# GrumpyZhou/patch2pix

Hardware: AMD Instinct MI355X
Metric: image-pairs/sec (480x640, ptmax=400), matching hot path, feature pyramids resident in HBM (higher is better)
Workload: dtype f32-equivalent: fp16x2 (every f32 operand, scaled by an exact power of two, = sum of 2 fp16 planes to within 2^-24 of its magnitude; 3 fp16 MFMA products per f32 product, f32 accumulate); second convolution as Winograd F(2x2,3x3) (transforms in f32, filters transformed in f64)

## Files before the change

### patch2pix_amd/csrc/regress_common.h

```cpp
#pragma once
#include "p2p_common.h"
#include <algorithm>
#include <cmath>
#include <cstring>
#include <vector>

namespace p2p {

constexpr int NT = 512;
constexpr int MAXB = 16;

struct RegDev {
    const float *wp1, *wp2;
    const float *wh1, *wh2;
    const float *bn1s, *bn1b, *bn2s, *bn2b;
    const float *bn1s_h, *bn2s_h;
    const float *fc1t, *fc1b, *bnf1s, *bnf1b, *fc2t, *fc2b, *bnf2s, *bnf2b, *fc3, *fc3b;
    const float *fc1p, *fc2p;
    const float *ww2, *bn2s_w;
};

struct ItemDev {
    const float *pyr[2][4];
    int H[2], W[2];
};

struct RegressArgs {
    ItemDev item[MAXB];
    int start[MAXB + 1];
    const int *dev_counts;
    int nitems;
    const void *proposals;
    int is_float, n, nlevels;
    RegDev reg[2];
    float *matches[2], *probs[2], *raw[2];
    float *ws;
    unsigned char *wU;
    float *hinv;
    int lvl0, p0, p1, mblocks;
};
static_assert(sizeof(RegDev) == 24 * sizeof(void *) && sizeof(RegressArgs) == 1864, "kernel-argument layout of the fine stage");

constexpr int FC_ROWS = 16;
constexpr int WINO_BLK = 16384;
#ifndef P2P_WINO_CHUNK
#define P2P_WINO_CHUNK 3328
#endif
constexpr int WINO_CHUNK = P2P_WINO_CHUNK;
static_assert(WINO_CHUNK % 256 == 0 && WINO_CHUNK >= 256, "chunks are whole units of 256 proposals");
static inline int wino_nchunks(size_t n) {
    const size_t units = (n + 255) / 256, per = WINO_CHUNK / 256;
    return (int)std::max<size_t>(1, (units + per - 1) / per);
}
static inline void wino_chunk_range(size_t n, int c, int *p0, int *p1) {
    const size_t units = (n + 255) / 256, nch = (size_t)wino_nchunks(n), base = units / nch, rem = units % nch;
    const size_t u0 = (size_t)c * base + std::min<size_t>((size_t)c, rem), u1 = u0 + base + ((size_t)c < rem ? 1 : 0);
    *p0 = (int)std::min(n, u0 * 256);
    *p1 = (int)std::min(n, u1 * 256);
}
static inline size_t regress_ws_base_floats(size_t n) { return ((2 * n * 512 + 31) & ~size_t(31)) + 4 * n + 32; }
static inline size_t wino_hinv_offset_floats(size_t n) { return (regress_ws_base_floats(n) + 63) & ~size_t(63); }
static inline size_t wino_chunk_rows(size_t n) {
    return (std::min(n, (size_t)WINO_CHUNK) + 7) & ~size_t(7);
}
static inline size_t wino_u_offset_floats(size_t n) { return (wino_hinv_offset_floats(n) + wino_chunk_rows(n) + 63) & ~size_t(63); }
static inline size_t regress_ws_floats(size_t n) {
    return wino_u_offset_floats(n) + (size_t)16 * (wino_chunk_rows(n) / 8) * 16 * (WINO_BLK / 4);
}

__device__ __forceinline__ int clampi(int v, int lo, int hi) { return v < lo ? lo : (v > hi ? hi : v); }

__device__ __forceinline__ int level_dim(int dim, int j) { return (dim + (1 << j) - 1) >> j; }

__device__ __forceinline__ int patch_cell(int origin, int p, int j, int dim) {
    const int d = dim >> j;
    return clampi((origin + p) >> j, 0, d - 1) - clampi(origin >> j, 0, d - 1);
}

template <class A>
__device__ __forceinline__ int wino_slot(const A &a, int c) {
    if (!a.dev_counts) return c < a.n ? c : -1;
    int cum = 0;
    for (int it = 0; it < a.nitems; ++it) {
        const int cnt = max(0, min(a.dev_counts[it], a.start[it + 1] - a.start[it]));
        if (c < cum + cnt) return a.start[it] + (c - cum);
        cum += cnt;
    }
    return -1;
}

__device__ __forceinline__ void fc_tail_parse(const RegDev &R, const ItemDev &I, const RegressArgs &args, int lvl, int prop,
                                              int tid, const float *V, float *F1, float *F2, float *misc) {
    P2P_OPAQUE(tid);
    {
        const f32x4 *w = (const f32x4 *)R.fc1t + tid;
        float s = 0.f;
#pragma unroll 1
        for (int k0 = 0; k0 < 128; k0 += 32) {
            f32x4 wv[32];
#pragma unroll
            for (int i = 0; i < 32; ++i) wv[i] = w[(k0 + i) * 512];
#pragma unroll
            for (int i = 0; i < 32; ++i) {
                const f32x4 x = *(const f32x4 *)(V + 4 * (k0 + i));
                s = fmaf(wv[i][0], x[0], s);
                s = fmaf(wv[i][1], x[1], s);
                s = fmaf(wv[i][2], x[2], s);
                s = fmaf(wv[i][3], x[3], s);
            }
        }
        s += R.fc1b[tid];
        F1[tid] = fmaxf(fmaf(s, R.bnf1s[tid], R.bnf1b[tid]), 0.f);
    }
    __syncthreads();
    if (tid < 256) {
        const f32x4 *w = (const f32x4 *)R.fc2t + tid;
        float s = 0.f;
#pragma unroll 1
        for (int k0 = 0; k0 < 128; k0 += 32) {
            f32x4 wv[32];
#pragma unroll
            for (int i = 0; i < 32; ++i) wv[i] = w[(k0 + i) * 256];
#pragma unroll
            for (int i = 0; i < 32; ++i) {
                const f32x4 x = *(const f32x4 *)(F1 + 4 * (k0 + i));
                s = fmaf(wv[i][0], x[0], s);
                s = fmaf(wv[i][1], x[1], s);
                s = fmaf(wv[i][2], x[2], s);
                s = fmaf(wv[i][3], x[3], s);
            }
        }
        s += R.fc2b[tid];
        F2[tid] = fmaxf(fmaf(s, R.bnf2s[tid], R.bnf2b[tid]), 0.f);
    }
    __syncthreads();
    if (tid < 5) {
        const f32x4 *w = (const f32x4 *)(R.fc3 + tid * 256);
        float s = 0.f;
#pragma unroll 1
        for (int k0 = 0; k0 < 64; k0 += 16) {
            f32x4 wv[16];
#pragma unroll
            for (int i = 0; i < 16; ++i) wv[i] = w[k0 + i];
#pragma unroll
            for (int i = 0; i < 16; ++i) {
                const f32x4 x = *(const f32x4 *)(F2 + 4 * (k0 + i));
                s = fmaf(wv[i][0], x[0], s);
                s = fmaf(wv[i][1], x[1], s);
                s = fmaf(wv[i][2], x[2], s);
                s = fmaf(wv[i][3], x[3], s);
            }
        }
        s += R.fc3b[tid];
        misc[tid] = s;
        if (args.raw[lvl]) args.raw[lvl][(size_t)prop * 5 + tid] = s;
        if (tid < 4) {
            const float off = 16.0f * tanhf(fmaxf(s, 0.f)) - 8.0f;
            float fm = misc[8 + tid] + off;
            const float hi = (float)((tid == 0) ? I.W[0] : (tid == 1) ? I.H[0] : (tid == 2) ? I.W[1] : I.H[1]);
            fm = fminf(fmaxf(fm, 0.f), hi);
            if (args.matches[lvl]) args.matches[lvl][(size_t)prop * 4 + tid] = fm;
            misc[8 + tid] = fm;
        } else {
            if (args.probs[lvl]) args.probs[lvl][prop] = 1.0f / (1.0f + expf(-s));
        }
    }
    __syncthreads();
}

__device__ __forceinline__ float load_coherent(const float *p) {
    return __int_as_float(__atomic_load_n((const int *)p, __ATOMIC_RELAXED));
}
#define P2P_MFMA_F32_16(a, b, c) __builtin_amdgcn_mfma_f32_16x16x4f32((a), (b), (c), 0, 0, 0)

constexpr int FCST1 = 512 + 4, FCST2 = 256 + 4;
constexpr int FC_LDS_BYTES = FC_ROWS * (2 * FCST1 + FCST2) * 4;

__device__ __forceinline__ void fc_batch_parse(const RegDev &R, const RegressArgs &args, int lvl, const float *wsV,
                                               float *nextp, unsigned char *smb, int tid) {
    P2P_OPAQUE(tid);
    const int nwg = gridDim.x, first = blockIdx.x;
    const int cnt = (args.n - first + nwg - 1) / nwg;
    const int lane = tid & 63, wave = __builtin_amdgcn_readfirstlane(tid >> 6), l15 = lane & 15, kb = lane >> 4;
    float *Vs = (float *)smb, *F1s = Vs + FC_ROWS * FCST1, *F2s = F1s + FC_ROWS * FCST1;
#pragma unroll 1
    for (int r0 = 0; r0 < cnt; r0 += FC_ROWS) {
        {
            const int row = tid >> 5, c4 = tid & 31;
            const bool ok = r0 + row < cnt;
            const float *src = wsV + (size_t)(first + (r0 + row) * nwg) * 512;
#pragma unroll
            for (int q = 0; q < 4; ++q) {
                const int col = 4 * (c4 + 32 * q);
                f32x4 v = {0.f, 0.f, 0.f, 0.f};
                if (ok) v = (f32x4){load_coherent(src + col), load_coherent(src + col + 1), load_coherent(src + col + 2), load_coherent(src + col + 3)};
                *(f32x4 *)(Vs + row * FCST1 + col) = v;
            }
        }
        __syncthreads();
        {
            f32x4 acc[4];
#pragma unroll
            for (int t = 0; t < 4; ++t) acc[t] = (f32x4){0.f, 0.f, 0.f, 0.f};
            const float *w = R.fc1p + ((size_t)(wave * 4) * 64 + lane) * 4;
            const float *a = Vs + l15 * FCST1 + 4 * kb;
#pragma unroll 2
            for (int S = 0; S < 32; ++S) {
                const f32x4 av = *(const f32x4 *)(a + 16 * S);
                f32x4 bv[4];
#pragma unroll
                for (int t = 0; t < 4; ++t) bv[t] = *(const f32x4 *)(w + ((size_t)S * 32 + t) * 256);
#pragma unroll
                for (int j = 0; j < 4; ++j)
#pragma unroll
                    for (int t = 0; t < 4; ++t) acc[t] = P2P_MFMA_F32_16(av[j], bv[t][j], acc[t]);
            }
#pragma unroll
            for (int t = 0; t < 4; ++t) {
                const int n = 16 * (4 * wave + t) + l15;
                const float b = R.fc1b[n], s = R.bnf1s[n], sh = R.bnf1b[n];
#pragma unroll
                for (int r = 0; r < 4; ++r) F1s[(4 * kb + r) * FCST1 + n] = fmaxf(fmaf(acc[t][r] + b, s, sh), 0.f);
            }
        }
        __syncthreads();
        {
            f32x4 acc[2];
#pragma unroll
            for (int t = 0; t < 2; ++t) acc[t] = (f32x4){0.f, 0.f, 0.f, 0.f};
// ... 184 lines not shown
```

### patch2pix_amd/csrc/regress_h2.hip

```cpp
#define XNPL 2
#include "regress_common.h"

#include <algorithm>
#include <cmath>
#include <vector>

namespace p2p {

typedef _Float16 xe8 __attribute__((ext_vector_type(8)));
typedef _Float16 xe2 __attribute__((ext_vector_type(2)));
typedef float f32x2 __attribute__((ext_vector_type(2)));
constexpr int XUB = XNPL * 1024;

constexpr int XST1 = 64 * 2 + 16;
constexpr int XRP1 = 9 * XST1 + 112;
constexpr int XPL1 = 9 * XRP1;
constexpr int YST2 = 64 * 2 + 16, YNC2 = 25, YPL2 = (YNC2 + 3) * YST2;
constexpr int YST3 = 128 * 2 + 32, YNC3 = 9, YPL3 = (YNC3 + 2) * YST3;
constexpr int XOFF1 = 0;
constexpr int YOFF2 = XOFF1 + XNPL * XPL1;
constexpr int YOFF3 = YOFF2 + XNPL * YPL2;
constexpr int XIMG = YOFF3 + XNPL * YPL3;
constexpr int XRAW0 = 2 * XIMG;
constexpr int XSHARED = XRAW0 + 2 * 3 * 256 * 4;
// ... 16 lines not shown
#ifdef P2P_X3_TIMING
constexpr int XSM_BYTES = XSM_MISC + 16 * 4 + 8 * 16 * 4;
#else
constexpr int XSM_BYTES = XSM_MISC + 16 * 4;
#endif
static_assert(FC_LDS_BYTES <= XSM_MISC, "the FC batch stages its rows over the convolution buffers");
static_assert(XTMP1 + 2 * XTMP1IMG <= XSHR && 64 * XA0ST <= XSHR, "the shared region is sized by the fold buffers");
static_assert(XPL1 % 16 == 0 && XTMP1 % 16 == 0 && XIMG % 16 == 0 && YOFF2 % 16 == 0 && YOFF3 % 16 == 0 && YPL2 % 16 == 0 && YPL3 % 16 == 0 && XSHARED % 16 == 0 &&
              XTAB % 16 == 0 && XSM_SCALE % 16 == 0 && HPL % 16 == 0 && HCHUNK % 16 == 0 && XCONV2B % 16 == 0,
              "16-byte alignment of ds_read_b128");
static_assert(XSM_BYTES <= 160 * 1024, "LDS budget");

__device__ __forceinline__ unsigned pk_e(float a, float b) {
    const f32x2 v = {a, b};
    return __builtin_bit_cast(unsigned, __builtin_convertvector(v, xe2));
}
__device__ __forceinline__ unsigned short f2e(float f) { return __builtin_bit_cast(unsigned short, (_Float16)f); }
__device__ __forceinline__ float e2f(unsigned short b) { return (float)__builtin_bit_cast(_Float16, b); }
__device__ __forceinline__ float pk_lo(unsigned h) { return (float)__builtin_bit_cast(xe2, h)[0]; }
__device__ __forceinline__ float pk_hi(unsigned h) { return (float)__builtin_bit_cast(xe2, h)[1]; }
__device__ __forceinline__ void store_planes(unsigned char *dst, int plane_stride, float v) {
    const unsigned short p0 = f2e(v);
    const float r1 = v - e2f(p0);
    const unsigned short p1 = f2e(r1);
    *(unsigned short *)dst = p0;
    *(unsigned short *)(dst + plane_stride) = p1;
}

__device__ __forceinline__ void splitn(const f32x4 &xa, const f32x4 &xb, float s, f32x4 (&p)[XNPL]) {
    const float x[8] = {xa[0] * s, xa[1] * s, xa[2] * s, xa[3] * s, xb[0] * s, xb[1] * s, xb[2] * s, xb[3] * s};
#pragma unroll
    for (int q = 0; q < 4; ++q) {
        const unsigned h = pk_e(x[2 * q], x[2 * q + 1]);
        const float r0 = x[2 * q] - pk_lo(h);
        const float r1 = x[2 * q + 1] - pk_hi(h);
        const unsigned m = pk_e(r0, r1);
        p[0][q] = __uint_as_float(h);
        p[1][q] = __uint_as_float(m);
    }
}

#ifdef XF_PIN_W
#define XWADV(N)
#else
#define XWADV(N) wb += (N) * XUB;
#endif
#ifdef P2P_X3_TIMING
#define XTL_() ((unsigned *)(smb + XSM_MISC + 64) + wave * 16)
#define XT_START { const unsigned n_ = (unsigned)__builtin_amdgcn_s_memtime(); if (P2P_LANE_ID() < 16) XTL_()[P2P_LANE_ID()] = (P2P_LANE_ID() == 15) ? n_ : 0u; }
#define XT(i) { const unsigned n_ = (unsigned)__builtin_amdgcn_s_memtime(); if (P2P_LANE_ID() == 0) { unsigned *x_ = XTL_(); x_[i] += n_ - x_[15]; x_[15] = n_; } }
#if P2P_X3_TIMING >= 2
#define XTL(i) XT(i)
#else
#define XTL(i)
#endif
#else
#define XT_START
#define XT(i)
#define XTL(i)
#endif
#define XMFMA(a, b, c) __builtin_amdgcn_mfma_f32_32x32x16_f16(__builtin_bit_cast(xe8, (a)), __builtin_bit_cast(xe8, (b)), (c), 0, 0, 0)

#define XLOADR(R, P) R[0] = *(const f32x4 *)(P); R[1] = *(const f32x4 *)((P) + 16);
#define XLOADP(S, P, PL) { _Pragma("unroll") for (int q_ = 0; q_ < XNPL; ++q_) S[q_] = *(const f32x4 *)((P) + q_ * (PL)); }
#define XLOADB(BUF, AHEAD)                                                               \
    { unsigned wo_ = (AHEAD) * XUB; P2P_OPAQUE_S(wo_);          \
      _Pragma("unroll") for (int q_ = 0; q_ < XNPL; ++q_) BUF[q_] = *(const f32x4 *)((wb + wo_) + wlane + q_ * 1024); }
#define XNPROD 3
#define XHALF_(C0IN, C1IN, CU0, CU1, SP, BU0, BU1)                                       \
    CU0 = XMFMA(SP[1], BU0[0], C0IN); CU1 = XMFMA(SP[1], BU1[0], C1IN);                  \
    CU0 = XMFMA(SP[0], BU0[1], CU0); CU1 = XMFMA(SP[0], BU1[1], CU1);                    \
    CU0 = XMFMA(SP[0], BU0[0], CU0); CU1 = XMFMA(SP[0], BU1[0], CU1);
#define XNM (2 * XNPROD)
#define XHALF(CU0, CU1, SP, BU0, BU1) XHALF_(CU0, CU1, CU0, CU1, SP, BU0, BU1)
#define XHALFZ(CU0, CU1, SP, BU0, BU1) XHALF_(zero16, zero16, CU0, CU1, SP, BU0, BU1)

#define XPIPE(NDS)                                                                       \
    __builtin_amdgcn_sched_group_barrier(0x100, NDS, 0); __builtin_amdgcn_sched_group_barrier(0x020, XNPL, 0);        \
    _Pragma("unroll") for (int g_ = 0; g_ < XNM; ++g_) {                                                              \
        __builtin_amdgcn_sched_group_barrier(0x008, 1, 0); __builtin_amdgcn_sched_group_barrier(0x002, 6, 0); }
#define XPIPE0()                                                                         \
    __builtin_amdgcn_sched_group_barrier(0x020, XNPL, 0);                                                             \
    _Pragma("unroll") for (int g_ = 0; g_ < XNM; ++g_) {                                                              \
        __builtin_amdgcn_sched_group_barrier(0x008, 1, 0); __builtin_amdgcn_sched_group_barrier(0x002, 6, 0); }
#define XSLAB(N0, N1, SC0, SC1, BC0, BC1, BN0, BN1, AH)                                   \
    { XLOADR(R0, N0) XLOADB(BN0, AH) splitn(R1[0], R1[1], (SC1), S1);                               \
      XHALF(acc00, acc01, S0, BC0, BC1) XPIPE(2) __builtin_amdgcn_sched_barrier(0);                                   \
      XLOADR(R1, N1) XLOADB(BN1, (AH) + 1) splitn(R0[0], R0[1], (SC0), S0);                          \
      XHALF(acc10, acc11, S1, BC0, BC1) XPIPE(2) __builtin_amdgcn_sched_barrier(0); }
#define XGROUP4(SL0, SL1, SL2, SL3) { SL0 SL1 SL2 SL3 XWADV(8) }
#define XSLABEND(SC1, BC0, BC1, BN0, BN1, AH)                                            \
    { XLOADB(BN0, AH) splitn(R1[0], R1[1], (SC1), S1);                                              \
      XHALF(acc00, acc01, S0, BC0, BC1) XPIPE0() __builtin_amdgcn_sched_barrier(0);                                    \
      XLOADB(BN1, (AH) + 1)                                                                                           \
      XHALF(acc10, acc11, S1, BC0, BC1) XPIPE0() __builtin_amdgcn_sched_barrier(0); }
#define XPRO(P0, P1, SC0) { XLOADR(R0, P0) XLOADR(R1, P1) splitn(R0[0], R0[1], (SC0), S0); }

#define XQHALF_(C0IN, C1IN, CU0, CU1, A0, A1, BU)                                        \
    CU0 = XMFMA(A0[1], BU[0], C0IN); CU1 = XMFMA(A1[1], BU[0], C1IN);                    \
    CU0 = XMFMA(A0[0], BU[1], CU0); CU1 = XMFMA(A1[0], BU[1], CU1);                      \
    CU0 = XMFMA(A0[0], BU[0], CU0); CU1 = XMFMA(A1[0], BU[0], CU1);
#define XQHALF(CU0, CU1, A0, A1, BU) XQHALF_(CU0, CU1, CU0, CU1, A0, A1, BU)
#define XQHALFZ(CU0, CU1, A0, A1, BU) XQHALF_(zero16, zero16, CU0, CU1, A0, A1, BU)
#define XQPIPE()                                                                         \
    _Pragma("unroll") for (int g_ = 0; g_ < 2 * XNPL; ++g_) {                                                        \
        __builtin_amdgcn_sched_group_barrier(0x008, 1, 0); __builtin_amdgcn_sched_group_barrier(0x100, 1, 0); }       \
    __builtin_amdgcn_sched_group_barrier(0x008, 1, 0); __builtin_amdgcn_sched_group_barrier(0x020, XNPL, 0);          \
    __builtin_amdgcn_sched_group_barrier(0x008, 1, 0);
#define XQSTEP(HALF, AC0, AC1, AN0, AN1, NP0, NP1, BC, BN, AH)                            \
    { XLOADP(AN0, NP0, XPL1) XLOADP(AN1, NP1, XPL1) XLOADB(BN, AH)                                                    \
      HALF(tp0, tp1, AC0, AC1, BC) XQPIPE() __builtin_amdgcn_sched_barrier(0); }
#define XPFOLD(ACC0, ACC1)                                                               \
    { _Pragma("unroll") for (int r_ = 0; r_ < 16; ++r_) {                                                             \
          const float e0_ = *(const float *)(tabq + ((2 * (r_ >> 2)) * 17 + 2 * (r_ & 3)) * 8);                       \
          const float e1_ = *(const float *)(tabq + ((8 + 2 * (r_ >> 2)) * 17 + 2 * (r_ & 3)) * 8);                   \
          ACC0[r_] = fmaf(e0_, tp0[r_], ACC0[r_]); ACC1[r_] = fmaf(e1_, tp1[r_], ACC1[r_]); } }

#define XLPIPE(NDS, NMFMA)                                                               \
    __builtin_amdgcn_sched_group_barrier(0x100, NDS, 0); __builtin_amdgcn_sched_group_barrier(0x020, 2 * XNPL, 0);    \
    __builtin_amdgcn_sched_group_barrier(0x008, NMFMA, 0);
#define XCSLAB(HALF, SC, SN, NP, NPL, BC0, BC1, BN0, BN1, AH)                             \
    { XLOADP(SN, NP, NPL) XLOADB(BN0, AH) XLOADB(BN1, (AH) + 1)                                                       \
      HALF(t0, t1, SC, BC0, BC1) XLPIPE(XNPL, XNM) __builtin_amdgcn_sched_barrier(0); }
typedef float f32x4v __attribute__((ext_vector_type(4)));
#define X16MFMA(a, b, c) __builtin_amdgcn_mfma_f32_16x16x32_f16(__builtin_bit_cast(xe8, (a)), __builtin_bit_cast(xe8, (b)), (c), 0, 0, 0)
#define X16HALF_(C0IN, C1IN, CU0, CU1, SP, BU0, BU1)                                     \
    CU0 = X16MFMA(SP[1], BU0[0], C0IN); CU1 = X16MFMA(SP[1], BU1[0], C1IN);              \
    CU0 = X16MFMA(SP[0], BU0[1], CU0); CU1 = X16MFMA(SP[0], BU1[1], CU1);                \
    CU0 = X16MFMA(SP[0], BU0[0], CU0); CU1 = X16MFMA(SP[0], BU1[0], CU1);
#define X16HALF(CU0, CU1, SP, BU0, BU1) X16HALF_(CU0, CU1, CU0, CU1, SP, BU0, BU1)
#define X16HALFZ(CU0, CU1, SP, BU0, BU1) X16HALF_(zero4, zero4, CU0, CU1, SP, BU0, BU1)
#define X16SLAB(HALF, UA, UB, SC, LOADNEXT, BC0, BC1, BN0, BN1, AH)                       \
    { LOADNEXT XLOADB(BN0, AH) XLOADB(BN1, (AH) + 1)                                                                  \
      HALF(UA, UB, SC, BC0, BC1) __builtin_amdgcn_sched_barrier(0); }
#define XPB() { __builtin_amdgcn_sched_barrier(0); __builtin_amdgcn_s_barrier(); __builtin_amdgcn_sched_barrier(0); }
#define XPP() __builtin_amdgcn_sched_barrier(0); __builtin_amdgcn_s_barrier(); __builtin_amdgcn_s_barrier(); __builtin_amdgcn_sched_barrier(0);
#define XHPIPE()                                                                         \
    __builtin_amdgcn_sched_group_barrier(0x008, 2, 0);                                                                \
    _Pragma("unroll") for (int g_ = 0; g_ < 2 * XNPL; ++g_) {                                                        \
        __builtin_amdgcn_sched_group_barrier(0x100, 1, 0); __builtin_amdgcn_sched_group_barrier(0x008, 1, 0); }       \
    _Pragma("unroll") for (int g_ = 0; g_ < 2 * XNPL; ++g_) {                                                        \
        __builtin_amdgcn_sched_group_barrier(0x020, 1, 0); __builtin_amdgcn_sched_group_barrier(0x008, 1, 0); }       \
    __builtin_amdgcn_sched_group_barrier(0x008, 4 * XNPROD - 4 * XNPL - 2, 0);
#define XQUAD(AC0, AC1, BC0, BC1, P, Q)                                                  \
    acc00 = XMFMA(AC0[P], BC0[Q], acc00); acc01 = XMFMA(AC0[P], BC1[Q], acc01);                                       \
    acc11 = XMFMA(AC1[P], BC1[Q], acc11); acc10 = XMFMA(AC1[P], BC0[Q], acc10);
#define XHMFMAS(AC0, AC1, BC0, BC1)                                                      \
    XQUAD(AC0, AC1, BC0, BC1, 1, 0) XQUAD(AC0, AC1, BC0, BC1, 0, 1) XQUAD(AC0, AC1, BC0, BC1, 0, 0)
#define XHSLAB(AC0, AC1, AN0, AN1, NP0, NP1, BC0, BC1, BN0, BN1, AH)                       \
    { XLOADP(AN0, NP0, HPL) XLOADP(AN1, NP1, HPL) XLOADB(BN0, AH) XLOADB(BN1, (AH) + 1)                                \
      XHMFMAS(AC0, AC1, BC0, BC1)                                                                                     \
      XHPIPE() __builtin_amdgcn_sched_barrier(0); }

enum : int {
    MISC_NEXT_PROP = 4,
    MISC_PROP = 8,
    MISC_MIN_SCALE = 12,
    MISC_MAX_H = 14,
};
static_assert(MISC_MAX_H == MISC_MIN_SCALE + 2, "the three reductions are reset by three consecutive threads");

__device__ __forceinline__ int image_exponent(const float *misc, int img) {
    return clampi((((const int *)misc)[MISC_MIN_SCALE + img] >> 23) & 0xff, 13, 240);
}
__device__ __forceinline__ int h_exponent(const float *misc) { return clampi((((const int *)misc)[MISC_MAX_H] >> 23) & 0xff, 20, 250); }
__device__ __forceinline__ float cell_mul(int eb) { return __int_as_float((eb + 12) << 23); }
__device__ __forceinline__ float fold_mul(int eb) { return __int_as_float((254 - eb) << 23); }
__device__ __forceinline__ float h_mul(int eb, int top) { return __int_as_float((254 + top - eb) << 23); }
__device__ __forceinline__ float h_inv(int eb, int top) { return __int_as_float((eb - top) << 23); }

constexpr int level_cells(int j) { return (j == 0) ? 16 : (j == 1) ? 9 : (j == 2) ? 5 : 3; }
constexpr int level_channels(int j) { return (j == 0) ? 3 : (j == 3) ? 128 : 64; }
constexpr int level_loads(int j) { return (level_channels(j) * level_cells(j) * level_cells(j) + NT - 1) / NT; }
__device__ __forceinline__ int tmp_cell(int img, int j, int c) {
    return (j == 1) ? XSHARED + XTMP1 + img * XTMP1IMG + c * XTMP1ST
                    : XSHARED + img * XTMPIMG + ((j == 2) ? c * XTMP2ST : XTMP3 + c * XTMP3ST);
}
__device__ __forceinline__ int opaque_tid(int wave) {
    int t = wave * 64 + P2P_LANE_ID();
    P2P_OPAQUE(t);
    return t;
}
struct GatherRegs { float v[2][4][level_loads(1)]; };
__device__ __forceinline__ void gather_loads(GatherRegs &g, int tv, int xa, int ya, int xb, int yb, const ItemDev &J) {
#pragma unroll
    for (int img = 0; img < 2; ++img) {
        const int Hh = J.H[img], Ww = J.W[img], x0 = img ? xb : xa, y0 = img ? yb : ya;
        {
            const int r0 = clampi(y0, 0, Hh - 1), c0 = clampi(x0, 0, Ww - 1);
            const float *src = J.pyr[img][0];
#pragma unroll
            for (int k = 0; k < level_loads(0); ++k) {
                const int e = tv + k * NT;
                const int c = e >> 8, rem = e & 255, r = rem >> 4, cc = rem & 15;
                g.v[img][0][k] = (e < 768) ? src[((size_t)c * Hh + min(r0 + r, Hh - 1)) * Ww + min(c0 + cc, Ww - 1)] : 0.f;
            }
        }
#pragma unroll
        for (int j = 1; j < 4; ++j) {
            const int Rr = level_cells(j);
            const int Hj = Hh >> j, Wj = Ww >> j;
            const int Ha = level_dim(Hh, j), Wa = level_dim(Ww, j);
            const int r0 = clampi(y0 >> j, 0, Hj - 1);
            const int c0 = clampi(x0 >> j, 0, Wj - 1);
            const float *src = J.pyr[img][j];
#pragma unroll
            for (int k = 0; k < level_loads(j); ++k) {
                const int e = tv + k * NT;
                const int c = e / (Rr * Rr);
                const int rem = e - c * (Rr * Rr);
                const int r = rem / Rr;
                const int cc = rem - r * Rr;
                g.v[img][j][k] = (e < level_channels(j) * Rr * Rr)
                                     ? src[((size_t)c * Ha + min(r0 + r, Hj - 1)) * Wa + min(c0 + cc, Wj - 1)] : 0.f;
            }
        }
    }
}
__device__ __forceinline__ void gather_commit(const GatherRegs &g, int tv, unsigned char *smb) {
#pragma unroll
    for (int img = 0; img < 2; ++img) {
#pragma unroll
        for (int k = 0; k < level_loads(0); ++k) {
            const int e = tv + k * NT;
            if (e < 768) ((float *)(smb + XRAW0))[img * 768 + e] = g.v[img][0][k];
        }
#pragma unroll
        for (int j = 1; j < 4; ++j) {
            const int Rr = level_cells(j);
#pragma unroll
            for (int k = 0; k < level_loads(j); ++k) {
                const int e = tv + k * NT;
                if (e < level_channels(j) * Rr * Rr) {
                    const int c = e / (Rr * Rr);
                    const int rem = e - c * (Rr * Rr);
                    *(float *)(smb + tmp_cell(img, j, rem) + c * 4) = g.v[img][j][k];
                }
            }
        }
    }
}
__device__ __forceinline__ void gather_zero(GatherRegs &g) {
    float zf = 0.f;
    P2P_OPAQUE(zf);
#pragma unroll
    for (int img = 0; img < 2; ++img)
#pragma unroll
        for (int j = 0; j < 4; ++j)
#pragma unroll
            for (int k = 0; k < level_loads(j); ++k) g.v[img][j][k] = zf;
}

#define XWS_V(lvl_) (args.ws + (size_t)(lvl_) * args.n * 512)
#define XWS_NEXTP() (args.ws + ((2 * (size_t)args.n * 512 + 31) & ~(size_t)31))
__device__ __forceinline__ float proposal_coord(const RegressArgs &args, int lvl, int prop, int q) {
    if (lvl > 0) return load_coherent(XWS_NEXTP() + (size_t)prop * 4 + q);
    if (args.is_float) return ((const float *)args.proposals)[(size_t)prop * 4 + q];
    return (float)((const long long *)args.proposals)[(size_t)prop * 4 + q];
}

template <bool WINO>
__global__ __launch_bounds__(NT, 2) void regress_h2_kernel(RegressArgs args) {
    P2P_DYN_SHARED(unsigned char, smb);
    const int tid = threadIdx.x;
    const int wave = __builtin_amdgcn_readfirstlane(tid >> 6);
    const int nwg = gridDim.x;

    float *raw0 = (float *)(smb + XRAW0);
    float *scale = (float *)(smb + XSM_SCALE);
    float *misc = (float *)(smb + XSM_MISC);

#pragma unroll 1
    for (int lvl = WINO ? args.lvl0 : 0; lvl < (WINO ? args.lvl0 + 1 : args.nlevels); ++lvl) {
        const RegDev &R_ = args.reg[lvl];
        GatherRegs gn;
        bool pre = false;
#pragma unroll 1
      for (int cprop = (WINO ? args.p0 : 0) + blockIdx.x; cprop < (WINO ? args.p1 : args.n); cprop += nwg) {
        const int prop = WINO ? wino_slot(args, cprop) : cprop;
        if (WINO && prop < 0) break;
        int it = 0;
        while (it + 1 < args.nitems && prop >= args.start[it + 1]) ++it;
        if (!WINO && args.dev_counts && prop - args.start[it] >= args.dev_counts[it]) continue;
        const ItemDev &I = args.item[it];
        int tq = tid;
        if constexpr (WINO) tq = opaque_tid(wave);
        if (tq < 4) {
            float v = proposal_coord(args, lvl, prop, tq);
#ifdef XF_SAME_PATCH
            v = 100.f + 16.f * tq;
#endif
            misc[MISC_PROP + tq] = v;
        }
        if constexpr (WINO) {
            const int nprop = (cprop + nwg < args.p1) ? wino_slot(args, cprop + nwg) : -1;
            if (nprop >= 0 && tq >= 4 && tq < 8) misc[MISC_NEXT_PROP + tq - 4] = proposal_coord(args, lvl, nprop, tq - 4);
        }
        if (tq >= 64 && tq < 67) ((int *)misc)[MISC_MIN_SCALE + tq - 64] = (tq < 66) ? 0x7f7fffff : 0;
        __syncthreads();
        int moff = MISC_PROP;
        P2P_OPAQUE(moff);
        const int xa = (int)misc[moff + 0] - 8, ya = (int)misc[moff + 1] - 8;
        const int xb = (int)misc[moff + 2] - 8, yb = (int)misc[moff + 3] - 8;
#define XX0(img_) ((img_) ? xb : xa)
#define XY0(img_) ((img_) ? yb : ya)
        const int tidv = opaque_tid(wave);
        const int half = (tidv >> 5) & 1, l31 = tidv & 31;
        XT_START
        if (wave >= 4) __builtin_amdgcn_s_setprio(1);

        if constexpr (WINO) {
            if (!pre) gather_loads(gn, opaque_tid(wave), xa, ya, xb, yb, I);
            gather_commit(gn, opaque_tid(wave), smb);
        } else {
            GatherRegs g;
            gather_loads(g, tidv, xa, ya, xb, yb, I);
            gather_commit(g, tidv, smb);
        }
        if (tidv < 2 * XNPL * (3 * YST2 + 2 * YST3) / 16) {
            const int per = (3 * YST2 + 2 * YST3) / 16;
            const int im = tidv / (XNPL * per), pl = (tidv / per) % XNPL, q = tidv % per;
            float zf = 0.f;
            P2P_OPAQUE(zf);
            unsigned char *z = smb + im * XIMG + ((q < 3 * YST2 / 16) ? YOFF2 + pl * YPL2 + YNC2 * YST2 + q * 16
                                                                      : YOFF3 + pl * YPL3 + YNC3 * YST3 + (q - 3 * YST2 / 16) * 16);
            *(f32x4 *)z = (f32x4){zf, zf, zf, zf};
        }
        __syncthreads();
        XT(0)

        float sc_keep;
        int c23_keep;
        {
            const int img = tidv >> 8, pix = tidv & 255, py = pix >> 4, px = pix & 15;
            float ss = 0.f;
            {
                const float *p = raw0 + img * 768 + patch_cell(XY0(img), py, 0, I.H[img]) * 16 + patch_cell(XX0(img), px, 0, I.W[img]);
#pragma unroll
                for (int c = 0; c < 3; ++c) ss = fmaf(p[c * 256], p[c * 256], ss);
            }
            const int c2 = patch_cell(XY0(img), py, 2, I.H[img]) * 5 + patch_cell(XX0(img), px, 2, I.W[img]);
#pragma unroll
            for (int j = 1; j < 4; ++j) {
                const int cjy = patch_cell(XY0(img), py, j, I.H[img]), cjx = patch_cell(XX0(img), px, j, I.W[img]);
                const unsigned char *p = smb + tmp_cell(img, j, cjy * level_cells(j) + cjx);
                for (int c = 0; c < level_channels(j); c += 4) {
                    const f32x4 v = *(const f32x4 *)(p + c * 4);
                    ss = fmaf(v[0], v[0], ss); ss = fmaf(v[1], v[1], ss); ss = fmaf(v[2], v[2], ss); ss = fmaf(v[3], v[3], ss);
                }
            }
            const float sc = 1.0f / sqrtf(ss + 1e-6f);
            scale[tidv] = sc * 4096.0f;
            atomicMin((int *)misc + MISC_MIN_SCALE + img, __float_as_int(sc));
            sc_keep = sc;
            c23_keep = c2 * XTROW | (patch_cell(XY0(img), py, 3, I.H[img]) * 3 + patch_cell(XX0(img), px, 3, I.W[img])) * XTROW << 16;
            if (tidv < 2 * 33) {
                const int im = tidv / 33, q = tidv - im * 33;
                const int idx = (q < 17) ? q : (q - 16) * 17;
                float zf = 0.f;
                P2P_OPAQUE(zf);
                *(f32x2 *)(smb + XTAB + im * XTABIMG + idx * 8) = (f32x2){zf, zf};
            }
        }
        __syncthreads();
        {
            const int img = tidv >> 8, pix = tidv & 255, py = pix >> 4, px = pix & 15;
            *(f32x2 *)(smb + XTAB + img * XTABIMG + ((py + 1) * 17 + px + 1) * 8) =
                (f32x2){sc_keep * fold_mul(image_exponent(misc, img)), __int_as_float(c23_keep)};
#pragma unroll
            for (int k = 0; k < 11; ++k) {
                const int e = tidv + k * NT;
                if (e < 2 * 2592) {
                    const int im = (e >= 2592), r = e - im * 2592;
                    const float mul = cell_mul(image_exponent(misc, im));
                    const int cell = r >> 5, c2 = (r & 31) * 2, cy = cell / 9, cx = cell - 9 * cy;
                    const f32x2 v = *(const f32x2 *)(smb + tmp_cell(im, 1, cell) + c2 * 4);
                    const unsigned h = pk_e(v[0] * mul, v[1] * mul);
                    unsigned char *d = smb + im * XIMG + XOFF1 + cy * XRP1 + cx * XST1 + c2 * 2;
                    *(unsigned *)d = h;
                    *(unsigned *)(d + XPL1) = pk_e(v[0] * mul - pk_lo(h), v[1] * mul - pk_hi(h));
                }
            }
#pragma unroll
            for (int k = 0; k < 11; ++k) {
                const int e = tidv + k * NT;
                if (e < 2 * 2752) {
                    const int im = (e >= 2752), r = e - im * 2752;
                    const float mul = cell_mul(image_exponent(misc, im));
                    const bool l2 = r < 1600;
                    const int cell = l2 ? r >> 6 : (r - 1600) >> 7, c = l2 ? r & 63 : (r - 1600) & 127;
                    const float v = *(const float *)(smb + tmp_cell(im, l2 ? 2 : 3, cell) + c * 4);
                    store_planes(smb + im * XIMG + (l2 ? YOFF2 + cell * YST2 : YOFF3 + cell * YST3) + c * 2, l2 ? YPL2 : YPL3, v * mul);
                }
            }
        }
        __syncthreads();
        XT(1)

        for (int e = tidv; e < 64 * 64; e += NT) {
            const int m = e >> 6, kk = e & 63, img = kk >> 5, r = kk & 31;
            float v = 0.f;
            if (r < 27) {
                const int tap = r / 3, c = r - tap * 3, ky = tap / 3, kx = tap - ky * 3;
                const int py = 2 * (m >> 3) + ky - 1, px = 2 * (m & 7) + kx - 1;
                if (py >= 0 && px >= 0)
                    v = raw0[img * 768 + c * 256 + patch_cell(XY0(img), py, 0, I.H[img]) * 16 + patch_cell(XX0(img), px, 0, I.W[img])] *
                        scale[img * 256 + py * 16 + px];
            }
            *(float *)(smb + XSHARED + m * XA0ST + kk * 4) = v;
        }
        __syncthreads();
        XT(2)

#define XZERO16(A_) { float z_ = 0.f; P2P_OPAQUE(z_); _Pragma("unroll") for (int i_ = 0; i_ < 16; ++i_) A_[i_] = z_; }
        f32x16 acc00, acc01, acc10, acc11;
        XZERO16(acc00) XZERO16(acc01) XZERO16(acc10) XZERO16(acc11)
        f32x4 B0[XNPL], B1[XNPL], B2[XNPL], B3[XNPL], B4[XNPL], B5[XNPL], B6[XNPL], B7[XNPL], S0[XNPL], S1[XNPL];
        const f32x16 zero16 = {0};
        auto acc_tile = [&](int t, int u) -> const f32x16 & { return (t == 0) ? (u == 0 ? acc00 : acc01) : (u == 0 ? acc10 : acc11); };
        auto bn1_absmax = [&]() {
            float mx = 0.f;
#pragma unroll
            for (int u = 0; u < 2; ++u) {
                const int n = wave * 64 + u * 32 + l31;
                const float s = R_.bn1s_h[n], b = R_.bn1b[n];
#pragma unroll
                for (int t = 0; t < 2; ++t) {
                    const f32x16 &a = acc_tile(t, u);
#pragma unroll
                    for (int r = 0; r < 16; ++r) mx = fmaxf(mx, fabsf(fmaf(a[r], s, b)));
                }
            }
            atomicMax((int *)misc + MISC_MAX_H, __float_as_int(mx));
        };
        {
            f32x4 R0[2], R1[2];
            const unsigned char *wb = (const unsigned char *)R_.wh1 + (size_t)wave * (S1_UNITS + XPF) * XUB;
            const unsigned wlane = (tidv & 63) * 16;
            XLOADB(B0, 0) XLOADB(B1, 1) XLOADB(B2, 2) XLOADB(B3, 3) XLOADB(B4, 4) XLOADB(B5, 5)
            {
                const unsigned char *p0 = smb + XSHARED + l31 * XA0ST + half * 32;
                const unsigned char *p1 = p0 + 32 * XA0ST;
                XPRO(p0, p1, 1.0f)
                XGROUP4(XSLAB(p0 + 64, p1 + 64, 1.0f, 1.0f, B0, B1, B6, B7, 6),
                        XSLAB(p0 + 128, p1 + 128, 1.0f, 1.0f, B2, B3, B0, B1, 8),
                        XSLAB(p0 + 192, p1 + 192, 1.0f, 1.0f, B4, B5, B2, B3, 10),
                        XSLAB(p0, p1, 1.0f, 1.0f, B6, B7, B4, B5, 12))
            }
            __syncthreads();
            XT(3)
            const int c2y = (l31 < 25) ? l31 / 5 : 0, c2x = (l31 < 25) ? l31 - 5 * (l31 / 5) : 0;
            float *Tw = (float *)(smb + XSHARED + (wave & (XT2N - 1)) * XTW) + 2 * l31;
            float *T3w = (float *)(smb + XSHARED + XT2N * XTW + wave * (9 * XTROW));
            const f32x4v zero4 = {0.f, 0.f, 0.f, 0.f};
            const int stagger = wave >> 2;
#pragma unroll 1
            for (int it = 0; it < 18 + stagger; ++it) {
                const int pi = it - stagger;
                if (pi >= 0) {
                    const int tap = pi >> 1, img = pi & 1;
                    const int ky = tap / 3, kx = tap - ky * 3;
                    int ab[2];
#pragma unroll
                    for (int t = 0; t < 2; ++t) {
                        const int p = 32 * t + l31;
                        const int pyc = max(2 * (p >> 3) + ky - 1, 0), pxc = max(2 * (p & 7) + kx - 1, 0);
                        ab[t] = img * XIMG + XOFF1 + patch_cell(XY0(img), pyc, 1, I.H[img]) * XRP1 +
                                patch_cell(XX0(img), pxc, 1, I.W[img]) * XST1 + half * 16;
                    }
                    const unsigned char *a0 = smb + ab[0], *a1 = smb + ab[1];
                    const unsigned char *tabq = smb + XTAB + img * XTABIMG + (ky * 17 + kx + 8 * half) * 8;
#ifdef XF_SKIP_P
                    XWADV(8) (void)a0; (void)a1; (void)tabq;
#else
                    {
                        f32x16 tp0, tp1;
                        XLOADP(S0, a0, XPL1) XLOADP(S1, a1, XPL1)
                        XQSTEP(XQHALFZ, S0, S1, R0, R1, a0 + 32, a1 + 32, B0, B6, 6)
                        XQSTEP(XQHALF, R0, R1, S0, S1, a0 + 64, a1 + 64, B1, B7, 7)
                        XQSTEP(XQHALF, S0, S1, R0, R1, a0 + 96, a1 + 96, B2, B0, 8)
                        XQSTEP(XQHALF, R0, R1, S0, S1, a0, a1, B3, B1, 9)
                        XPFOLD(acc00, acc10)
                        XQSTEP(XQHALFZ, S0, S1, R0, R1, a0 + 32, a1 + 32, B4, B2, 10)
                        XQSTEP(XQHALF, R0, R1, S0, S1, a0 + 64, a1 + 64, B5, B3, 11)
                        XQSTEP(XQHALF, S0, S1, R0, R1, a0 + 96, a1 + 96, B6, B4, 12)
                        XQSTEP(XQHALF, R0, R1, S0, S1, a0 + 96, a1 + 96, B7, B5, 13)
                        XPFOLD(acc01, acc11)
                        XWADV(8)
                    }
#endif
                    XTL(4)
                }
                if (it < 18) {
                    const int tap = it >> 1, img = it & 1;
                    const int ky = tap / 3, kx = tap - ky * 3;
                    int a2, a3;
                    {
                        const int Hh = I.H[img], Ww = I.W[img];
                        const int by2 = clampi(XY0(img) >> 2, 0, (Hh >> 2) - 1), bx2 = clampi(XX0(img) >> 2, 0, (Ww >> 2) - 1);
                        const int by3 = clampi(XY0(img) >> 3, 0, (Hh >> 3) - 1), bx3 = clampi(XX0(img) >> 3, 0, (Ww >> 3) - 1);
                        const int c3y = clampi(min((by2 + c2y) >> 1, (Hh >> 3) - 1) - by3, 0, 2);
                        const int c3x = clampi(min((bx2 + c2x) >> 1, (Ww >> 3) - 1) - bx3, 0, 2);
                        a2 = img * XIMG + YOFF2 + ((l31 < 25) ? (c2y * 5 + c2x) * YST2 + half * 16
                                                              : YNC2 * YST2 + ((((l31 - YNC2) * 9 + half) & 15) << 4));
                        a3 = img * XIMG + YOFF3 + ((l31 < 25) ? c3y * 3 + c3x : YNC3) * YST3 + half * 16;
                    }
                    const unsigned char *q2 = smb + a2, *q3 = smb + a3;
                    f32x16 t0, t1;
#if defined(XF_SKIP_C)
                    t0 = acc00; t1 = acc01; XWADV(24) (void)q2; (void)q3;
#else
                    {
                        (void)q3;
                        const int l16 = (tidv & 15), kb = (tidv >> 4) & 3;
                        const unsigned char *q3r = smb + img * XIMG + YOFF3 + ((l16 < 9) ? l16 * YST3 + kb * 16
                                                                                         : YNC3 * YST3 + (((2 * (l16 - YNC3) + kb) & 15) << 4));
                        f32x4v u0, u1, u2, u3;
                        XLOADP(S0, q3r, YPL3)
                        XGROUP4(X16SLAB(X16HALFZ, u0, u1, S0, XLOADP(S1, q3r + 64, YPL3), B0, B1, B6, B7, 6),
                                X16SLAB(X16HALFZ, u2, u3, S0, , B2, B3, B0, B1, 8),
                                X16SLAB(X16HALF, u0, u1, S1, XLOADP(S0, q3r + 128, YPL3), B4, B5, B2, B3, 10),
                                X16SLAB(X16HALF, u2, u3, S1, , B6, B7, B4, B5, 12))
                        XGROUP4(X16SLAB(X16HALF, u0, u1, S0, XLOADP(S1, q3r + 192, YPL3), B0, B1, B6, B7, 6),
                                X16SLAB(X16HALF, u2, u3, S0, , B2, B3, B0, B1, 8),
                                X16SLAB(X16HALF, u0, u1, S1, XLOADP(S0, q2, YPL2), B4, B5, B2, B3, 10),
                                X16SLAB(X16HALF, u2, u3, S1, , B6, B7, B4, B5, 12))
                        P2P_WAVE_SYNC();
#pragma unroll
                        for (int r = 0; r < 4; ++r)
                            if (4 * kb + r < 9) {
                                f32x2 *d = (f32x2 *)(T3w + (4 * kb + r) * 64) + l16;
                                d[0] = (f32x2){u0[r], u2[r]}; d[16] = (f32x2){u1[r], u3[r]};
                            }
                        XGROUP4(XCSLAB(XHALFZ, S0, S1, q2 + 32, YPL2, B0, B1, B6, B7, 6),
                                XCSLAB(XHALF, S1, S0, q2 + 64, YPL2, B2, B3, B0, B1, 8),
                                XCSLAB(XHALF, S0, S1, q2 + 96, YPL2, B4, B5, B2, B3, 10),
                                XCSLAB(XHALF, S1, S0, q2 + 96, YPL2, B6, B7, B4, B5, 12))
                    }
#endif
                    XTL(5)
#ifndef XF_SKIP_FOLD
                    P2P_WAVE_SYNC();
#pragma unroll
                    for (int r = 0; r < 16; ++r) {
                        const int row = (r & 3) + 8 * (r >> 2);
                        if ((r < 12 || half == 0) && row + 4 * half < XTROWS) {
                            *(f32x2 *)(Tw + (row + 4 * half) * 64) = (f32x2){t0[r], t1[r]};
                        }
                    }
                    P2P_WAVE_SYNC();
                    {
                        const unsigned char *tabp = smb + XTAB + img * XTABIMG + (ky * 17 + kx + 8 * half) * 8;
                        const unsigned char *Tr = (const unsigned char *)Tw;
#pragma unroll
                        for (int t = 0; t < 2; ++t)
#pragma unroll
                            for (int r = 0; r < 16; ++r) {
                                const f32x2 e = *(const f32x2 *)(tabp + ((8 * t + 2 * (r >> 2)) * 17 + 2 * (r & 3)) * 8);
                                const int offs = __float_as_int(e[1]);
                                const f32x2 g = *(const f32x2 *)(Tr + (offs & 0xffff));
                                const f32x2 h3 = *(const f32x2 *)((const unsigned char *)(T3w + 2 * l31) + (offs >> 16));
                                const float v0 = g[0] + h3[0], v1 = g[1] + h3[1];
// ... 355 lines not shown
```

Baseline: 949.7.

## Precompute level-0 im2col gather table and vectorize fp16 plane packing

Level-0 im2col construction now reads a compile-time constant table of 16-bit shared-memory float indices held in device memory. Each thread loads 8 entries and writes two 16-byte vectors, replacing per-element tap and patch_cell arithmetic. Pixels are pre-scaled into raw0 in place, which drops the separate scale array. The level 1-3 fp16 two-plane packing loops are merged into one loop that handles 4 floats per element with 8-byte stores. The cost is an extra global table load per thread and a changed raw0 layout that later consumers must agree with.

```diff
diff --git a/patch2pix_amd/csrc/regress_common.h b/patch2pix_amd/csrc/regress_common.h
--- a/patch2pix_amd/csrc/regress_common.h
+++ b/patch2pix_amd/csrc/regress_common.h
@@ -75,6 +75,14 @@
 __device__ __forceinline__ int patch_cell(int origin, int p, int j, int dim) {
     const int d = dim >> j;
     return clampi((origin + p) >> j, 0, d - 1) - clampi(origin >> j, 0, d - 1);
+}
+
+constexpr int level0_im2col_source(int m, int kk) {
+    const int img = kk >> 5, r = kk & 31;
+    if (r >= 27) return -1;
+    const int tap = r / 3, c = r - tap * 3, ky = tap / 3, kx = tap - ky * 3;
+    const int py = 2 * (m >> 3) + ky - 1, px = 2 * (m & 7) + kx - 1;
+    return (py < 0 || px < 0) ? -1 : img * 768 + c * 256 + py * 16 + px;
 }
 
 template <class A>
diff --git a/patch2pix_amd/csrc/regress_h2.hip b/patch2pix_amd/csrc/regress_h2.hip
--- a/patch2pix_amd/csrc/regress_h2.hip
+++ b/patch2pix_amd/csrc/regress_h2.hip
@@ -192,6 +192,20 @@
       XHMFMAS(AC0, AC1, BC0, BC1)                                                                                     \
       XHPIPE() __builtin_amdgcn_sched_barrier(0); }
 
+struct alignas(16) XA0Tab { unsigned short v[64 * 64]; };
+constexpr XA0Tab make_a0_tab() {
+    XA0Tab t = {};
+    for (int m = 0; m < 64; ++m)
+        for (int kk = 0; kk < 64; ++kk) {
+            const int s = level0_im2col_source(m, kk);
+            t.v[m * 64 + kk] = (unsigned short)((s < 0) ? XTAB / 4 : XRAW0 / 4 + s);
+        }
+    return t;
+}
+static_assert(XTAB / 4 < 65536 && XRAW0 % 4 == 0 && XTAB % 4 == 0, "the entries are 16-bit float indices");
+__device__ const XA0Tab xa0_tab = make_a0_tab();
+constexpr int XQ1 = 81 * 16, XQ2 = YNC2 * 16, XQ3 = YNC3 * 32, XQIMG = XQ1 + XQ2 + XQ3;
+
 enum : int {
     MISC_NEXT_PROP = 4,
     MISC_PROP = 8,
@@ -307,7 +321,6 @@
     const int nwg = gridDim.x;
 
     float *raw0 = (float *)(smb + XRAW0);
-    float *scale = (float *)(smb + XSM_SCALE);
     float *misc = (float *)(smb + XSM_MISC);
 
 #pragma unroll 1
@@ -369,30 +382,30 @@
         __syncthreads();
         XT(0)
 
-        float sc_keep;
+        const uint4 a0t = *(const uint4 *)(xa0_tab.v + 8 * tidv);
+        float sc_keep, l0s[3];
         int c23_keep;
         {
             const int img = tidv >> 8, pix = tidv & 255, py = pix >> 4, px = pix & 15;
             float ss = 0.f;
-            {
-                const float *p = raw0 + img * 768 + patch_cell(XY0(img), py, 0, I.H[img]) * 16 + patch_cell(XX0(img), px, 0, I.W[img]);
-#pragma unroll
-                for (int c = 0; c < 3; ++c) ss = fmaf(p[c * 256], p[c * 256], ss);
-            }
+            const float *p = raw0 + img * 768 + patch_cell(XY0(img), py, 0, I.H[img]) * 16 + patch_cell(XX0(img), px, 0, I.W[img]);
+#pragma unroll
+            for (int c = 0; c < 3; ++c) ss = fmaf(p[c * 256], p[c * 256], ss);
             const int c2 = patch_cell(XY0(img), py, 2, I.H[img]) * 5 + patch_cell(XX0(img), px, 2, I.W[img]);
 #pragma unroll
             for (int j = 1; j < 4; ++j) {
                 const int cjy = patch_cell(XY0(img), py, j, I.H[img]), cjx = patch_cell(XX0(img), px, j, I.W[img]);
-                const unsigned char *p = smb + tmp_cell(img, j, cjy * level_cells(j) + cjx);
+                const unsigned char *pc = smb + tmp_cell(img, j, cjy * level_cells(j) + cjx);
                 for (int c = 0; c < level_channels(j); c += 4) {
-                    const f32x4 v = *(const f32x4 *)(p + c * 4);
+                    const f32x4 v = *(const f32x4 *)(pc + c * 4);
                     ss = fmaf(v[0], v[0], ss); ss = fmaf(v[1], v[1], ss); ss = fmaf(v[2], v[2], ss); ss = fmaf(v[3], v[3], ss);
                 }
             }
             const float sc = 1.0f / sqrtf(ss + 1e-6f);
-            scale[tidv] = sc * 4096.0f;
             atomicMin((int *)misc + MISC_MIN_SCALE + img, __float_as_int(sc));
             sc_keep = sc;
+#pragma unroll
+            for (int c = 0; c < 3; ++c) l0s[c] = p[c * 256] * (sc * 4096.0f);
             c23_keep = c2 * XTROW | (patch_cell(XY0(img), py, 3, I.H[img]) * 3 + patch_cell(XX0(img), px, 3, I.W[img])) * XTROW << 16;
             if (tidv < 2 * 33) {
                 const int im = tidv / 33, q = tidv - im * 33;
@@ -408,46 +421,50 @@
             *(f32x2 *)(smb + XTAB + img * XTABIMG + ((py + 1) * 17 + px + 1) * 8) =
                 (f32x2){sc_keep * fold_mul(image_exponent(misc, img)), __int_as_float(c23_keep)};
 #pragma unroll
-            for (int k = 0; k < 11; ++k) {
+            for (int c = 0; c < 3; ++c) raw0[img * 768 + c * 256 + pix] = l0s[c];
+#pragma unroll
+            for (int k = 0; k < (2 * XQIMG + NT - 1) / NT; ++k) {
                 const int e = tidv + k * NT;
-                if (e < 2 * 2592) {
-                    const int im = (e >= 2592), r = e - im * 2592;
+                if (e < 2 * XQIMG) {
+                    const int im = (e >= XQIMG), r = e - im * XQIMG;
                     const float mul = cell_mul(image_exponent(misc, im));
-                    const int cell = r >> 5, c2 = (r & 31) * 2, cy = cell / 9, cx = cell - 9 * cy;
-                    const f32x2 v = *(const f32x2 *)(smb + tmp_cell(im, 1, cell) + c2 * 4);
-                    const unsigned h = pk_e(v[0] * mul, v[1] * mul);
-                    unsigned char *d = smb + im * XIMG + XOFF1 + cy * XRP1 + cx * XST1 + c2 * 2;
-                    *(unsigned *)d = h;
-                    *(unsigned *)(d + XPL1) = pk_e(v[0] * mul - pk_lo(h), v[1] * mul - pk_hi(h));
-                }
-            }
-#pragma unroll
-            for (int k = 0; k < 11; ++k) {
-                const int e = tidv + k * NT;
-                if (e < 2 * 2752) {
-                    const int im = (e >= 2752), r = e - im * 2752;
-                    const float mul = cell_mul(image_exponent(misc, im));
-                    const bool l2 = r < 1600;
-                    const int cell = l2 ? r >> 6 : (r - 1600) >> 7, c = l2 ? r & 63 : (r - 1600) & 127;
-                    const float v = *(const float *)(smb + tmp_cell(im, l2 ? 2 : 3, cell) + c * 4);
-                    store_planes(smb + im * XIMG + (l2 ? YOFF2 + cell * YST2 : YOFF3 + cell * YST3) + c * 2, l2 ? YPL2 : YPL3, v * mul);
+                    int src, dst, pls;
+                    if (r < XQ1) {
+                        const int cell = r >> 4, q = r & 15, cy = (cell * 57) >> 9;
+                        src = tmp_cell(im, 1, cell) + q * 16;
+                        dst = XOFF1 + cell * XST1 + cy * (XRP1 - 9 * XST1) + q * 8;
+                        pls = XPL1;
+                    } else if (r < XQ1 + XQ2) {
+                        const int cell = (r - XQ1) >> 4, q = (r - XQ1) & 15;
+                        src = tmp_cell(im, 2, cell) + q * 16;
+                        dst = YOFF2 + cell * YST2 + q * 8;
+                        pls = YPL2;
+                    } else {
+                        const int cell = (r - XQ1 - XQ2) >> 5, q = (r - XQ1 - XQ2) & 31;
+                        src = tmp_cell(im, 3, cell) + q * 16;
+                        dst = YOFF3 + cell * YST3 + q * 8;
+                        pls = YPL3;
+                    }
+                    const f32x4 v = *(const f32x4 *)(smb + src);
+                    const unsigned ha = pk_e(v[0] * mul, v[1] * mul), hb = pk_e(v[2] * mul, v[3] * mul);
+                    unsigned char *d = smb + im * XIMG + dst;
+                    *(uint2 *)d = make_uint2(ha, hb);
+                    *(uint2 *)(d + pls) = make_uint2(pk_e(v[0] * mul - pk_lo(ha), v[1] * mul - pk_hi(ha)),
+                                                     pk_e(v[2] * mul - pk_lo(hb), v[3] * mul - pk_hi(hb)));
                 }
             }
         }
         __syncthreads();
         XT(1)
 
-        for (int e = tidv; e < 64 * 64; e += NT) {
-            const int m = e >> 6, kk = e & 63, img = kk >> 5, r = kk & 31;
-            float v = 0.f;
-            if (r < 27) {
-                const int tap = r / 3, c = r - tap * 3, ky = tap / 3, kx = tap - ky * 3;
-                const int py = 2 * (m >> 3) + ky - 1, px = 2 * (m & 7) + kx - 1;
-                if (py >= 0 && px >= 0)
-                    v = raw0[img * 768 + c * 256 + patch_cell(XY0(img), py, 0, I.H[img]) * 16 + patch_cell(XX0(img), px, 0, I.W[img])] *
-                        scale[img * 256 + py * 16 + px];
-            }
-            *(float *)(smb + XSHARED + m * XA0ST + kk * 4) = v;
+        {
+            const unsigned t4[4] = {a0t.x, a0t.y, a0t.z, a0t.w};
+            float a[8];
+#pragma unroll
+            for (int i = 0; i < 8; ++i) a[i] = ((const float *)smb)[(t4[i >> 1] >> (16 * (i & 1))) & 0xffffu];
+            unsigned char *d = smb + XSHARED + (tidv >> 3) * XA0ST + (tidv & 7) * 32;
+            *(f32x4 *)d = (f32x4){a[0], a[1], a[2], a[3]};
+            *(f32x4 *)(d + 16) = (f32x4){a[4], a[5], a[6], a[7]};
         }
         __syncthreads();
         XT(2)
```

Result: no change. 956.1 (median of 6 runs) (+0.7%).
